# RazonIn4K/image-restoration-platform

Measured on AMD Instinct MI355X. Metric: restored images/sec @1024x1024 bs=8, higher is better.
Workload: dtype bf16; 1 GPU; 1024x1024 RGB u8, batch 8 per GPU: fused classifier scan + RestoreNet-v0 (43 convs, 779.9 GFLOP/image), seeded random-init weights; global_batch=8, parallelism=per-image data parallel x1, no collective, streams=1

## Files before the change

### image_restoration_platform_amd/csrc/conv_dnq.hip

```cpp
#include "conv_mfma.hpp"
#include "persist.hpp"

#include <type_traits>

namespace ire {

namespace {

typedef __bf16 bf16x8_t __attribute__((ext_vector_type(8)));
typedef __bf16 bf16x2_t __attribute__((ext_vector_type(2)));
typedef float f32x2_t __attribute__((ext_vector_type(2)));
typedef float f32x16_t __attribute__((ext_vector_type(16)));
typedef unsigned u32x4_t __attribute__((ext_vector_type(4)));

#ifndef DQ_ST
#define DQ_ST IRE_ST_LINE
#endif
#ifndef DQ_ABL
#define DQ_ABL 0
#endif

constexpr int DQ_THREADS = 512;
constexpr int DQ_TH = 16, DQ_TW = 32, DQ_IH = 17, DQ_IW = 33, DQ_NT = 128, DQ_NTL = 4;
constexpr int DQ_TILE_PIECES = 36;
// ... 42 lines not shown
}

template <int COUT>
__global__ __launch_bounds__(DQ_THREADS) void conv_dnq_kernel(ConvArgs a) {
    constexpr int NT = DQ_NT, NTL = DQ_NTL, C = COUT;
    __shared__ __attribute__((aligned(16))) unsigned char smem[DQ_LDS];
    const unsigned smem_lds = (unsigned)(size_t)(__attribute__((address_space(3))) unsigned char*)smem;
    const int tid = threadIdx.x;
    const int lane = tid & 63, wave = tid >> 6;
    const int r = lane & 31, h = lane >> 5;
    const int wv = __builtin_amdgcn_readfirstlane(wave);

    const int NKC = a.nkc;
    const int Cin = a.cin0;
    const int tiles_per_img = a.tiles_x * a.tiles_y;
    PersistCursor cursor(a.tiles_x, a.tiles_y, a.nimg, C / NT, 4 * NKC);
    const int n_items = cursor.my_items, S = cursor.S;
    if (S == 0) return;

    unsigned slotc[5];
#pragma unroll
    for (int d = 0; d < 5; ++d) {
        int l2 = lane;
        asm volatile("" : "+v"(l2));
        const int piece = d < 4 ? 4 * wv + d : 32 + (wv & 3);
        const int s = piece * 64 + l2, p = s >> 2, c8 = (s & 3) ^ ((p >> 2) & 3);
        const int py = p / DQ_IW, px = p - py * DQ_IW;
        slotc[d] = (unsigned)py | ((unsigned)px << 8) | ((unsigned)c8 << 16);
    }
    const char* const zeros = reinterpret_cast<const char*>(a.zeros);
    struct Plan { const void* src[10]; unsigned dst[10]; int n; };
// ... 256 lines not shown
```

### image_restoration_platform_amd/csrc/conv_down.hip

```cpp
#include "conv_mfma.hpp"
#include "persist.hpp"

namespace ire {

namespace {

typedef __bf16 bf16x8_t __attribute__((ext_vector_type(8)));
typedef __bf16 bf16x2_t __attribute__((ext_vector_type(2)));
typedef float f32x2_t __attribute__((ext_vector_type(2)));
typedef float f32x16_t __attribute__((ext_vector_type(16)));
typedef unsigned u32x4_t __attribute__((ext_vector_type(4)));

#ifndef DN_LD_NT
#define DN_LD_NT 0
#endif
constexpr int DN_THREADS = 512;
constexpr int DN_TH = 16, DN_TW = 32;
constexpr int DN_IH = DN_TH + 1, DN_IW = DN_TW + 1;
constexpr int DN_IN_CHUNKS = DN_IH * DN_IW * 4;
constexpr int DN_IN_ITERS = (DN_IN_CHUNKS + DN_THREADS - 1) / DN_THREADS;
constexpr int DN_IN_BYTES = DN_IN_ITERS * DN_THREADS * 16;
constexpr int DN_NT = 64, DN_NTL = 2;
constexpr int DN_W_BYTES_MAX = 4 * 4 * DN_NT * 16;
constexpr int DN_W_BASE = 2 * DN_IN_BYTES;
// ... 30 lines not shown
template <int N> __device__ __forceinline__ void dn_wait_vm(bool counted) {
    if (counted) asm volatile("s_waitcnt vmcnt(%0)" :: "n"(N) : "memory");
    else asm volatile("s_waitcnt vmcnt(0)" ::: "memory");
}

__global__ __launch_bounds__(DN_THREADS) void conv_down_kernel(ConvArgs a) {
    __shared__ __attribute__((aligned(16))) unsigned char smem[DN_LDS];
    const unsigned smem_lds = (unsigned)(size_t)(__attribute__((address_space(3))) unsigned char*)smem;
    const int tid = threadIdx.x;
    const int lane = tid & 63, wave = tid >> 6;
    const int r = lane & 31, h = lane >> 5;
    const int c8_fixed = tid & 3;

    const int tiles_per_img = a.tiles_x * a.tiles_y;
    const int nkc = a.nkc;
    PersistCursor cursor(a.tiles_x, a.tiles_y, a.nimg, a.nblocks, 4 * nkc);
    const int my_items = cursor.my_items;
    const int S = cursor.S;
    if (S == 0) return;
    using StageInfo = PersistStage;
    StageInfo sq0 = cursor.cur, sq1 = cursor.next(), sq2 = cursor.next();

    const int Cin = a.cin0;
    const int cin_shift = 31 - __builtin_clz(Cin);

    int a_off[2][4];
#pragma unroll
    for (int m = 0; m < 2; ++m)
#pragma unroll
        for (int o = 0; o < 4; ++o) {
            const int dy = (o >> 1) - 1, dx = (o & 1) - 1;
// ... 258 lines not shown
```

### image_restoration_platform_amd/csrc/conv_f8.hip

```cpp
#include "conv_mfma.hpp"
#include "persist.hpp"
#include "gn_fold.hpp"

namespace ire {

namespace {

typedef __bf16 bf16x2_t __attribute__((ext_vector_type(2)));
typedef float f32x2_t __attribute__((ext_vector_type(2)));
typedef float f32x16_t __attribute__((ext_vector_type(16)));
typedef unsigned u32x4_t __attribute__((ext_vector_type(4)));
typedef int i32x8_t __attribute__((ext_vector_type(8)));

constexpr float kF8ActScale = 16.0f;
constexpr int F8_THREADS = 512;
constexpr int F8_TH = 16, F8_TW = 32, F8_IH = 18, F8_IW = 34;
constexpr int F8_PX = F8_IH * F8_IW;
constexpr int F8_IN_CHUNKS = F8_PX * 4;
constexpr int F8_IN_ITERS = (F8_IN_CHUNKS + F8_THREADS - 1) / F8_THREADS;
constexpr int F8_PLANE = F8_PX * 16;
constexpr int F8_IN_BYTES = 2 * F8_PLANE + 64;
constexpr int F8_NT = 128, F8_NTL = 4;
constexpr int F8_W_BYTES = 9 * 2 * F8_NT * 16;
constexpr int F8_W_CHUNKS = F8_W_BYTES / 16;
// ... 35 lines not shown
}

struct F8Regs { uint4 v[F8_IN_ITERS]; unsigned ok; };

template <bool RESID>
__global__ __launch_bounds__(F8_THREADS) void conv_f8_kernel(ConvArgs a) {
    __shared__ __attribute__((aligned(16))) unsigned char smem[F8_LDS];
    const unsigned smem_lds = (unsigned)(size_t)(__attribute__((address_space(3))) unsigned char*)smem;
    const int tid = threadIdx.x;
    const int lane = tid & 63, wave = tid >> 6;
    const int r = lane & 31, h = lane >> 5;
    const int c8_fixed = tid & 3;

    const int tiles_per_img = a.tiles_x * a.tiles_y;
    const int nkc = a.nkc;
    PersistCursor cursor(a.tiles_x, a.tiles_y, a.nimg, a.nblocks, nkc);
    const int my_items = cursor.my_items;
    const int S = cursor.S;
    if (S == 0) return;
    if (a.gn_stats) gn_fold(a, smem, cursor.first_img, cursor.last_img);
    using StageInfo = PersistStage;
    StageInfo sq0 = cursor.cur, sq1 = cursor.next(), sq2 = cursor.next();

    const int Cin = a.cin0;
    const int cin_shift = 31 - __builtin_clz(Cin);

    int p_off[2][5], w_off[5];
#pragma unroll
    for (int i = 0; i < 5; ++i) {
        const int tap = min(2 * i + h, 8);
        const int ky = tap / 3, kx = tap - ky * 3;
// ... 291 lines not shown
```

### image_restoration_platform_amd/csrc/conv_mfma.hpp

```cpp
#pragma once
#include "common.hpp"
#include "conv_kind.hpp"

#ifndef IRE_ST_LINE
#define IRE_ST_LINE 16
#endif
#ifndef IRE_LD_ONCE
#define IRE_LD_ONCE 2
#endif
#ifndef IRE_LD_IN
#define IRE_LD_IN 0
#endif
#ifndef IRE_ST_PART
#define IRE_ST_PART 0
#endif

#include <cstdlib>

namespace ire {

inline int persistent_grid_cus() {
    static const int forced = [] { const char* v = std::getenv("IRE_GRID_CUS"); return v ? std::atoi(v) : 0; }();
    int dev = 0, cus = 256;
    (void)hipGetDevice(&dev);
// ... 25 lines not shown
    const unsigned char* u8_in;
    unsigned char* u8_out;
    float* stats;
    int Hin, Win, Hout, Wout, cout;
    int tiles_x, tiles_y, nimg, nblocks;
    int group_size;
    int prio_young;
    int in_rows;
    int in_row_off;
    int iy_lo, iy_span;
    int fp8;
    const float* oscale;
    int w4_nt;
    const void* zeros;
    unsigned long long* stamps;
};

void conv_launch(ConvKind kind, const ConvArgs& a, hipStream_t stream);

void conv_rb_launch(bool resid, bool fused_act, const ConvArgs& a, hipStream_t stream);
void conv_w4_launch(bool resid, const ConvArgs& a, hipStream_t stream);
void conv_f8_launch(bool resid, const ConvArgs& a, hipStream_t stream);
void conv_stem_launch(const ConvArgs& a, hipStream_t stream);
void conv_down_launch(const ConvArgs& a, hipStream_t stream);
void conv_head_launch(const ConvArgs& a, hipStream_t stream);
void conv_pc_launch(bool resid, bool head, const ConvArgs& a, hipStream_t stream);
void conv_pk_launch(bool resid, const ConvArgs& a, hipStream_t stream);
void conv_up_subpixel_launch(const ConvArgs& a, hipStream_t stream);
void conv_upq_launch(const ConvArgs& a, hipStream_t stream);
void conv_dnq_launch(const ConvArgs& a, hipStream_t stream);
// ... 4 lines not shown
```

### image_restoration_platform_amd/csrc/conv_pc.hip

```cpp
#include "conv_mfma.hpp"
#include "conv_plan.hpp"
#include "gn_fold.hpp"
#include "persist.hpp"

#include <type_traits>

namespace ire {

namespace {

typedef __bf16 bf16x8_t __attribute__((ext_vector_type(8)));
typedef __bf16 bf16x2_t __attribute__((ext_vector_type(2)));
typedef float f32x2_t __attribute__((ext_vector_type(2)));
typedef float f32x16_t __attribute__((ext_vector_type(16)));
typedef unsigned u32x4_t __attribute__((ext_vector_type(4)));

#ifndef C3_RES_PRE
#define C3_RES_PRE -1
#endif
#ifndef C3_SCALAR
#define C3_SCALAR 1
#endif
#ifndef C3_PRIO
#define C3_PRIO 1
// ... 89 lines not shown
        (void)k;
#endif
    };

    auto tl = [&](int slot) {
#ifdef IRE_W4_TL
        if (a.stamps && tid == 0) {
            a.stamps[(size_t)blockIdx.x * 32 + slot * 2] = __builtin_amdgcn_s_memrealtime();
            a.stamps[(size_t)blockIdx.x * 32 + slot * 2 + 1] = __builtin_amdgcn_s_memtime();
        }
#else
        (void)slot;
#endif
    };
    const int tiles_per_img = a.tiles_x * a.tiles_y;
    PersistCursor cursor(a.tiles_x, a.tiles_y, a.nimg, K::NBLK, NKC);
    const int n_items = cursor.my_items;
    if (n_items == 0) return;
    const int n_stages = n_items * NKC;
    tl(0);
    {
        const unsigned char* ws = reinterpret_cast<const unsigned char*>(a.w);
        const unsigned wl = (unsigned)(size_t)(__attribute__((address_space(3))) unsigned char*)smem + K::W_OFF;
        constexpr int PIECES = NKC * K::W_STAGE_CHUNKS / 64;
        static_assert((NKC * K::W_STAGE_CHUNKS) % 64 == 0, "whole wave-instructions");
        const int wv = __builtin_amdgcn_readfirstlane(wave);
        for (int p = wv; p < PIECES; p += THREADS / 64) c3_glds16(ws + ((size_t)p * 64 + lane) * 16, wl + p * 1024);
    }
    if (a.gn_stats) gn_fold(a, smem, cursor.first_img, cursor.last_img, 512, reinterpret_cast<float2*>(smem + K::COEF_OFF));
    tl(1);

// ... 606 lines not shown
```

### image_restoration_platform_amd/csrc/conv_pk.hip

```cpp
#include "conv_mfma.hpp"
#include "conv_plan.hpp"
#include "gn_fold.hpp"
#include "persist.hpp"

#include <type_traits>

namespace ire {

namespace {

typedef __bf16 bf16x8_t __attribute__((ext_vector_type(8)));
typedef __bf16 bf16x2_t __attribute__((ext_vector_type(2)));
typedef float f32x2_t __attribute__((ext_vector_type(2)));
typedef float f32x16_t __attribute__((ext_vector_type(16)));
typedef unsigned u32x4_t __attribute__((ext_vector_type(4)));

#ifndef PK_PRIO
#define PK_PRIO 1
#endif
#ifndef PK_DMA_SPLIT
#define PK_DMA_SPLIT 1
#endif
#ifndef PK_BDEPTH
#define PK_BDEPTH 2
// ... 73 lines not shown
    return x + y;
}
__device__ __forceinline__ void pk_barrier() { asm volatile("s_waitcnt lgkmcnt(0)\n\ts_barrier" ::: "memory"); }

template <int C, bool RESID>
__global__ __launch_bounds__(PK_THREADS) void conv_pk_kernel(ConvArgs a) {
    using K = PkCfg<C>;
    constexpr int NKC = C / 16, NBLK = C / PK_NT, NT = PK_NT, NTL = PK_NTL;
    __shared__ __attribute__((aligned(16))) unsigned char smem[K::LDS];
    const unsigned smem_lds = (unsigned)(size_t)(__attribute__((address_space(3))) unsigned char*)smem;
    const int tid = threadIdx.x;
    const int lane = tid & 63, wave = tid >> 6;
    const int r = lane & 31, h = lane >> 5;

    const int tiles_per_img = a.tiles_x * a.tiles_y;
    PersistCursor cursor(a.tiles_x, a.tiles_y, a.nimg, NBLK, NKC);
    const int n_items = cursor.my_items, S = cursor.S;
    if (S == 0) return;
    auto stamp = [&](int role, int stage, int k) {
#ifdef PK_TICKS
        if (a.stamps && lane == 0 && blockIdx.x < 8 && stage < 32) a.stamps[(((size_t)blockIdx.x * 2 + role) * 32 + stage) * 4 + k] = __builtin_amdgcn_s_memtime();
#else
        (void)role; (void)stage; (void)k;
#endif
    };
    auto tl = [&](int slot) {
#ifdef IRE_W4_TL
        if (a.stamps && tid == 0) {
            a.stamps[(size_t)blockIdx.x * 32 + slot * 2] = __builtin_amdgcn_s_memrealtime();
            a.stamps[(size_t)blockIdx.x * 32 + slot * 2 + 1] = __builtin_amdgcn_s_memtime();
        }
// ... 460 lines not shown
```

### image_restoration_platform_amd/csrc/conv_rb.hip

```cpp
#include "conv_mfma.hpp"
#include "persist.hpp"
#include "gn_fold.hpp"

#include <cstdlib>

namespace ire {

namespace {

typedef __bf16 bf16x8_t __attribute__((ext_vector_type(8)));
typedef __bf16 bf16x2_t __attribute__((ext_vector_type(2)));
typedef float f32x2_t __attribute__((ext_vector_type(2)));
typedef float f32x16_t __attribute__((ext_vector_type(16)));
typedef unsigned u32x4_t __attribute__((ext_vector_type(4)));

constexpr int RB_TH = kRbTileH, RB_TW = 32;
constexpr int RB_WAVES = RB_TH / 2;
constexpr int RB_THREADS = RB_WAVES * 64;
constexpr int RB_IH = RB_TH + 2, RB_IW = RB_TW + 2;
constexpr int RB_IN_CHUNKS = RB_IH * RB_IW * 4;
constexpr int RB_IN_ITERS = (RB_IN_CHUNKS + RB_THREADS - 1) / RB_THREADS;
constexpr int RB_IN_BYTES = RB_IN_ITERS * RB_THREADS * 16;
constexpr int RB_NSTEPS = 18;

// ... 70 lines not shown

    const unsigned smem_lds = (unsigned)(size_t)(__attribute__((address_space(3))) unsigned char*)smem;
    const int tid = threadIdx.x;
    const int lane = tid & 63, wave = tid >> 6;
    const int r = lane & 31, h = lane >> 5;
    const int c8_fixed = tid & 3;
    auto stamp = [&](int s, int k) {
        if constexpr (DBG & 16) {
            const unsigned long long t = __builtin_amdgcn_s_memtime();
            if (a.stamps && lane == 0 && (wave == 0 || wave == 4) && blockIdx.x < 8 && s < 64)
                a.stamps[(((size_t)blockIdx.x * 2 + (wave >> 2)) * 64 + s) * 10 + k] = t;
        }
    };

    const int tiles_per_img = a.tiles_x * a.tiles_y;
    PersistCursor cursor(a.tiles_x, a.tiles_y, a.nimg, a.nblocks, a.nkc);
    const int nkc = a.nkc;
    const int S = cursor.S;
    if (S == 0) return;
    if (a.gn_stats) gn_fold(a, smem, cursor.first_img, cursor.last_img);
    using StageInfo = PersistStage;
    StageInfo sq0 = cursor.cur, sq1 = cursor.next(), sq2 = cursor.next();

    const unsigned short* src = reinterpret_cast<const unsigned short*>(a.in0);
    const int Cin = a.cin0;

    int a_off[2][9];
#pragma unroll
    for (int m = 0; m < 2; ++m)
#pragma unroll
        for (int tap = 0; tap < 9; ++tap) {
// ... 482 lines not shown
```

### image_restoration_platform_amd/csrc/conv_stem.hip

```cpp
#include "conv_mfma.hpp"

#include <type_traits>

namespace ire {

namespace {

typedef __bf16 bf16x8_t __attribute__((ext_vector_type(8)));
typedef __bf16 bf16x2_t __attribute__((ext_vector_type(2)));
typedef float f32x2_t __attribute__((ext_vector_type(2)));
typedef float f32x16_t __attribute__((ext_vector_type(16)));
typedef unsigned u32x4_t __attribute__((ext_vector_type(4)));

constexpr int ST_THREADS = 512, ST_TH = 16, ST_TW = 32, ST_IH = ST_TH + 2, ST_IW = ST_TW + 2;
constexpr int ST_RB = ST_IW * 3;
constexpr int ST_PW = ST_IW + 2;
constexpr int ST_ROW = ST_PW * 4;
constexpr int ST_ITERS = (ST_IH * ST_RB + ST_THREADS - 1) / ST_THREADS;

__device__ __forceinline__ unsigned st_pack(float a, float b) {
    f32x2_t f = {a, b};
    return __builtin_bit_cast(unsigned, __builtin_convertvector(f, bf16x2_t));
}
template <int N> __device__ __forceinline__ float st_ror_add(float v) {
// ... 18 lines not shown
    f32x16_t bias_acc;
#pragma unroll
    for (int i = 0; i < 16; ++i) bias_acc[i] = a.bias[16 * (i >> 3) + 8 * h + (i & 7)];
    const int foff = (2 * wave * ST_PW + r + 2 * h) * 4;
    for (int i = tid; i < 2 * ST_IH * ST_ROW / 2; i += ST_THREADS) reinterpret_cast<unsigned*>(&tile[0][0])[i] = 0u;
    __syncthreads();
    int spy[ST_ITERS], sb[ST_ITERS], spx[ST_ITERS], srel[ST_ITERS];
#pragma unroll
    for (int it = 0; it < ST_ITERS; ++it) {
        const int i = tid + it * ST_THREADS;
        spy[it] = i / ST_RB; sb[it] = i - spy[it] * ST_RB;
        spx[it] = sb[it] / 3;
        srel[it] = (spy[it] * a.Win + spx[it]) * 3 + (sb[it] - spx[it] * 3);
    }

    const int tiles_per_img = a.tiles_x * a.tiles_y, total = tiles_per_img * a.nimg;
    const unsigned char* in = reinterpret_cast<const unsigned char*>(a.in0);
    const bf16x2_t ones = __builtin_bit_cast(bf16x2_t, 0x3f803f80u);
    unsigned pv[ST_ITERS];
    auto request = [&](int item) {
        const int img = item / tiles_per_img, t = item - img * tiles_per_img;
        const int ty = t / a.tiles_x, tx = t - ty * a.tiles_x;
        const int iy0 = ty * ST_TH - 1, ix0 = tx * ST_TW - 1;
        const long long base = (((long long)img * a.in_rows + iy0 + a.in_row_off) * a.Win + ix0) * 3;
#pragma unroll
        for (int it = 0; it < ST_ITERS; ++it) {
            const bool ok = spy[it] < ST_IH && (unsigned)(iy0 + spy[it] - a.iy_lo) < (unsigned)a.iy_span && (unsigned)(ix0 + spx[it]) < (unsigned)a.Win;
            const unsigned v = in[ok ? base + srel[it] : 0];
            pv[it] = ok ? v : 0u;
        }
    };
    int par = 0;
    if ((int)blockIdx.x < total) request(blockIdx.x);
    for (int item = blockIdx.x; item < total; item += gridDim.x) {
        const int img = item / tiles_per_img, t = item - img * tiles_per_img;
        const int ty = t / a.tiles_x, tx = t - ty * a.tiles_x;
        unsigned short* tl = tile[par];
#pragma unroll
        for (int it = 0; it < ST_ITERS; ++it)
            if (spy[it] < ST_IH) tl[spy[it] * ST_ROW + spx[it] * 4 + (sb[it] - spx[it] * 3)] = (unsigned short)(__builtin_bit_cast(unsigned, (float)pv[it]) >> 16);
        if (item + (int)gridDim.x < total) request(item + gridDim.x);
        __syncthreads();
        const int ox = tx * ST_TW + r;
        char* obase = reinterpret_cast<char*>(a.out) + (size_t)img * a.Hout * a.Wout * 64;
        float gs[2][2] = {{0.f, 0.f}, {0.f, 0.f}}, gq[2][2] = {{0.f, 0.f}, {0.f, 0.f}};
#pragma unroll
        for (int m = 0; m < 2; ++m) {
            u32x4_t f[3];
#pragma unroll
            for (int ky = 0; ky < 3; ++ky) {
                const uint2* fp = reinterpret_cast<const uint2*>(tl + foff + (m + ky) * ST_ROW);
                const uint2 lo = fp[0], hi = fp[1];
                f[ky] = u32x4_t{lo.x, lo.y, hi.x, hi.y};
            }
            f32x16_t c = __builtin_amdgcn_mfma_f32_32x32x16_bf16(w0, __builtin_bit_cast(bf16x8_t, f[0]), bias_acc, 0, 0, 0);
            c = __builtin_amdgcn_mfma_f32_32x32x16_bf16(w1, __builtin_bit_cast(bf16x8_t, f[1]), c, 0, 0, 0);
// ... 68 lines not shown
```

### image_restoration_platform_amd/csrc/conv_up.hip

```cpp
#include "conv_mfma.hpp"
#include "persist.hpp"

#include <type_traits>

namespace ire {

namespace {

typedef __bf16 bf16x8_t __attribute__((ext_vector_type(8)));
typedef __bf16 bf16x2_t __attribute__((ext_vector_type(2)));
typedef float f32x2_t __attribute__((ext_vector_type(2)));
typedef float f32x16_t __attribute__((ext_vector_type(16)));
typedef unsigned u32x4_t __attribute__((ext_vector_type(4)));

#ifndef IRE_UP_TEPI
#define IRE_UP_TEPI 1
#endif
#ifndef IRE_UP_ABL
#define IRE_UP_ABL 0
#endif
constexpr int UP_THREADS = 512;
constexpr int UP_TH = 16, UP_TW = 32;
constexpr int UP_IH = UP_TH + 2, UP_IW = UP_TW + 2;
constexpr int UP_IN_CHUNKS = UP_IH * UP_IW * 4;
// ... 35 lines not shown
    if constexpr (I < N) { f(std::integral_constant<int, I>{}); up_static_for<I + 1, N>(f); }
}

using UpItem = PersistItem;
struct UpRegs { uint4 v[UP_IN_ITERS]; };

template <int NKS>
__global__ __launch_bounds__(UP_THREADS) void conv_up_kernel(ConvArgs a) {
    __shared__ __attribute__((aligned(16))) unsigned char smem[UP_LDS];
    const unsigned smem_lds = (unsigned)(size_t)(__attribute__((address_space(3))) unsigned char*)smem;
    const int tid = threadIdx.x;
    const int lane = tid & 63, wave = tid >> 6;
    const int r = lane & 31, h = lane >> 5;
    const int c8_fixed = tid & 3;

    PersistCursor cursor(a.tiles_x, a.tiles_y, a.nimg, a.nblocks, a.nkc);
    const int my_items = cursor.my_items;
    const int nkc = a.nkc;
    const int S = cursor.S;
    if (S == 0) return;
    using StageInfo = PersistStage;
    StageInfo sq0 = cursor.cur, sq1 = cursor.next(), sq2 = cursor.next();

    const int Cin = a.cin0;
    const int cin_shift = 31 - __builtin_clz(Cin);

    int a_off[2][9];
#pragma unroll
    for (int m = 0; m < 2; ++m)
#pragma unroll
        for (int tap = 0; tap < 9; ++tap) {
// ... 466 lines not shown
```

### image_restoration_platform_amd/csrc/conv_upq.hip

```cpp
#include "conv_mfma.hpp"
#include "persist.hpp"

#include <type_traits>

namespace ire {

namespace {

typedef __bf16 bf16x8_t __attribute__((ext_vector_type(8)));
typedef __bf16 bf16x2_t __attribute__((ext_vector_type(2)));
typedef float f32x2_t __attribute__((ext_vector_type(2)));
typedef float f32x16_t __attribute__((ext_vector_type(16)));
typedef unsigned u32x4_t __attribute__((ext_vector_type(4)));

#ifndef UQ_ST
#define UQ_ST IRE_ST_LINE
#endif
#ifndef UQ_DMA_SPAN
#define UQ_DMA_SPAN 32
#endif
#ifndef UQ_ABL
#define UQ_ABL 0
#endif

// ... 35 lines not shown
}

__global__ __launch_bounds__(UQ_THREADS) void conv_upq_kernel(ConvArgs a) {
    constexpr int NT = UQ_NT, NTL = UQ_NTL, C = UQ_NT;
    __shared__ __attribute__((aligned(16))) unsigned char smem[UQ_LDS];
    const unsigned smem_lds = (unsigned)(size_t)(__attribute__((address_space(3))) unsigned char*)smem;
    const int tid = threadIdx.x;
    const int lane = tid & 63, wave = tid >> 6;
    const int r = lane & 31, h = lane >> 5;
    const int wv = __builtin_amdgcn_readfirstlane(wave);

    const int NKC = a.nkc;
    const int NST = NKC;
    const int Cin = a.cin0;
    const int tiles_per_img = a.tiles_x * a.tiles_y;
    PersistCursor cursor(a.tiles_x, a.tiles_y, a.nimg, 4, NST);
    const int n_items = cursor.my_items, S = cursor.S;
    if (S == 0) return;

    unsigned slotc[5];
#pragma unroll
    for (int d = 0; d < 5; ++d) {
        int l2 = lane;
        asm volatile("" : "+v"(l2));
        const int piece = d < 4 ? 4 * wv + d : 32 + (wv & 3);
        const int s = piece * 64 + l2, p = s >> 2, c8 = (s & 3) ^ ((p >> 2) & 3);
        const int py = p / UQ_IW, px = p - py * UQ_IW;
        slotc[d] = (unsigned)py | ((unsigned)px << 8) | ((unsigned)c8 << 16);
    }
    const char* const zeros = reinterpret_cast<const char*>(a.zeros);
    struct Plan { const void* src[10]; unsigned dst[10]; int n; };
// ... 276 lines not shown
```

### image_restoration_platform_amd/csrc/conv_w4.hip

```cpp
#include "conv_mfma.hpp"
#include "persist.hpp"
#include "gn_fold.hpp"

#include <cstdlib>
#include <type_traits>

#ifndef W4_TEPI
#define W4_TEPI 1
#endif

namespace ire {

namespace {

typedef __bf16 bf16x8_t __attribute__((ext_vector_type(8)));
typedef __bf16 bf16x2_t __attribute__((ext_vector_type(2)));
typedef float f32x2_t __attribute__((ext_vector_type(2)));
typedef float f32x16_t __attribute__((ext_vector_type(16)));

constexpr int W4_TH = 16, W4_TW = 32, W4_IH = 18, W4_IW = 34;
constexpr int W4_IN_CHUNKS = W4_IH * W4_IW * 2;
constexpr int W4_IN_BYTES = (W4_IN_CHUNKS + 8) * 16;
constexpr int W4_NSTEPS = 9;

// ... 59 lines not shown
__global__ __launch_bounds__(WAVES * 64) void conv_w4_kernel(ConvArgs a) {
    static_assert(!FP8 || (FUSED && WAVES == 8), "fp8 operands: fused-activation 8-wave form only");
    using C = W4Cfg<NT, WAVES, FP8>;
    constexpr int EB = C::EB;
    using Regs = W4Regs<C::IN_ITERS>;
    constexpr int NTL = C::NTL;
    __shared__ __attribute__((aligned(16))) unsigned char smem[C::LDS_BYTES];
    const unsigned smem_lds = (unsigned)(size_t)(__attribute__((address_space(3))) unsigned char*)smem;

    const int tid = threadIdx.x;
    const int lane = tid & 63, wave = tid >> 6;
    const int r = lane & 31, h = lane >> 5;
    const int c8_fixed = tid & 1;

    const int tiles_per_img = a.tiles_x * a.tiles_y;
    PersistCursor cursor(a.tiles_x, a.tiles_y, a.nimg, a.nblocks, a.nkc);
    const int my_items = cursor.my_items;
    const int nkc = a.nkc;
    const int S = cursor.S;
    if (S == 0) return;
#ifdef IRE_W4_TL
    if (a.stamps && tid == 0) { a.stamps[(size_t)blockIdx.x * 32] = __builtin_amdgcn_s_memrealtime(); a.stamps[(size_t)blockIdx.x * 32 + 1] = __builtin_amdgcn_s_memtime(); }
#endif
    using StageInfo = PersistStage;
    StageInfo sq0 = cursor.cur, sq1 = cursor.next(), sq2 = cursor.next();

    const int Cin = a.cin0;
    const int cin_shift = 31 - __builtin_clz(Cin);

    constexpr int PLANE = C::PLANE;
    const int a_base = h * PLANE + (wave * C::MT * W4_IW + r) * EB;
// ... 606 lines not shown
```

### image_restoration_platform_amd/csrc/engine.cpp

```cpp
#include "engine.hpp"
#include "encode.hpp"

#include <chrono>
#include <cmath>
#include <cstdlib>
#include <cstring>
#include <fstream>

#include "gn.hpp"
#include "strips.hpp"
#include "weight_pack.hpp"
#include "grey_tables.inc"

namespace ire {

namespace {

const int kWidths[4] = {32, 64, 128, 256};
const int kFilmOff[4] = {0, 64, 192, 448};
const int kFilmDim = 960;

inline double now_s() {
    return std::chrono::duration<double>(std::chrono::steady_clock::now().time_since_epoch()).count();
}
// ... 17 lines not shown
    hipDeviceProp_t prop;
    IRE_HIP(hipGetDeviceProperties(&prop, device_));
    if (std::strncmp(prop.gcnArchName, "gfx950", 6) != 0)
        fail(IRE_ERR_UNAVAILABLE, std::string("service unavailable: device is ") + prop.gcnArchName +
                                      ", this engine is built for gfx950 (MI355X) only");
    if (cfg.precision != IRE_PRECISION_BF16 && cfg.precision != IRE_PRECISION_FP8) fail(IRE_ERR_INVALID_INPUT, "invalid precision");
    precision_ = cfg.precision;
    max_batch_ = cfg.max_batch > 0 ? cfg.max_batch : 8;
    if (max_batch_ > 64) fail(IRE_ERR_INVALID_INPUT, "invalid max_batch (1..64)");
    num_lanes_ = cfg.num_streams > 0 ? cfg.num_streams : 1;
    if (num_lanes_ > 16) num_lanes_ = 16;
    if (cfg.flags & ~(uint32_t)IRE_FLAG_RESULT_PNG_BASE64) fail(IRE_ERR_INVALID_INPUT, "invalid ire_config.flags (unknown bits set)");
    flags_ = cfg.flags;
    sw_ = ConvSwitches::from_env();
    cus_ = persistent_grid_cus();
    if (const char* v = std::getenv("IRE_RB_STAMPS")) {
        stamps_cout_ = std::atoi(v);
        stamps_resid_ = std::strchr(v, 'r') != nullptr;
    }
    if (const char* v = std::getenv("IRE_W4_TL")) stamps_tl_ = v;

    IRE_HIP(hipStreamCreateWithFlags(&main_stream_, hipStreamNonBlocking));
    for (auto& ev : ev_) IRE_HIP(hipEventCreate(&ev));
    IRE_HIP(hipEventCreateWithFlags(&fork_ev_, hipEventDisableTiming));
    IRE_HIP(hipEventCreateWithFlags(&busy_ev_, hipEventDisableTiming));
    lanes_.resize(num_lanes_);
    for (auto& L : lanes_) {
        IRE_HIP(hipStreamCreateWithFlags(&L.stream, hipStreamNonBlocking));
        IRE_HIP(hipEventCreateWithFlags(&L.done, hipEventDisableTiming));
    }
// ... 538 lines not shown
    a.cin0 = d.cin0; a.cin1 = p.cin1; a.kc_split = d.kc_split; a.nkc = p.nkc; a.nblocks = p.nblocks; a.w4_nt = p.w4_nt; a.fp8 = p.fp8;
    const unsigned short* const slabs[] = {nullptr, cw.d_w, cw.d_wp, cw.d_w4, cw.d_w4h, cw.d_wstem, cw.d_wd, cw.d_wu, cw.d_wuf, cw.d_wdq, cw.d_wuq, cw.d_wsq,
                                           cw.d_wsk, reinterpret_cast<const unsigned short*>(cw.d_w8x), reinterpret_cast<const unsigned short*>(cw.d_w8)};
    const float* const biases[] = {cw.d_bias, cw.d_bias_uf, cw.d_bias8};
    a.w = slabs[p.w]; a.w1 = slabs[p.w1]; a.bias = biases[p.bias];
    if (p.fp8) a.oscale = cw.d_oscale;
    if (p.zeros) a.zeros = d_zero_;
    a.ab = op.use_ab ? R.ab : nullptr; a.resid = out_ptr(op.resid); a.out = out_ptr(op.out);
    a.u8_in = d.kind == CONV_HEAD ? g.img_in + (size_t)g.halo * g.w * 3 : nullptr;
    a.u8_out = d.kind == CONV_HEAD ? g.img_out : nullptr;
    a.Hin = g.h >> op.lin; a.Win = g.w >> op.lin; a.Hout = Hout; a.Wout = Wout;
    a.in_rows = p.in_rows; a.in_row_off = p.in_row_off; a.iy_lo = p.iy_lo; a.iy_span = p.iy_span;
    a.cout = p.cout; a.group_size = p.group_size; a.tiles_x = p.tiles_x; a.tiles_y = p.tiles_y; a.nimg = g.nimg;
    if (op.stats_out) a.stats = (R.stats_alt ? R.stats_alt : R.stats) + p.stats_offset();
    a.prio_young = sw_.prio_young;
    const bool rb = d.kind == CONV_RB1 || d.kind == CONV_RB2;
    if (stamps_dev_ && rb && d.cout == stamps_cout_ && (d.kind == CONV_RB2) == stamps_resid_ && (!stamps_taken_ || !stamps_tl_.empty() || std::getenv("IRE_STAMPS_RAW"))) {
        a.stamps = stamps_dev_;
        stamps_taken_ = true;
    }
    if (R.gn_pending) {
        if (p.folds_gn) {
            const GNW& gn = *R.gn_pending;
            a.gn_stats = R.gn_stats; a.gn_parts = R.gn_parts; a.gn_hw = (g.H >> gn.level) * (g.w >> gn.level);
            a.gn_gamma = gn.d_gamma; a.gn_beta = gn.d_beta; a.gn_film = R.film; a.gn_film_stride = kFilmDim; a.gn_film_off = kFilmOff[gn.level];
            a.ab_w = R.ab;
            R.gn_pending = nullptr;
        } else flush_gn(R, g);
    }
    prof_begin(p.fam, R.stream, p.flops, p.bytes);
// ... 36 lines not shown

void Engine::exec_op(Run& R, const Op& op, const Geo& g) {
    switch (op.kind) {
        case Op::GN: {
            R.gn_pending = op.gn; R.gn_stats = R.stats; R.gn_parts = R.stat_parts;
            if (!sw_.gn_fold || g.halo) flush_gn(R, g);
            break;
        }
        case Op::CONV: exec_conv(R, op, g); break;
    }
}

void Engine::run_network(Lane& L, int nimg, int h, int w, const uint8_t* d_in, uint8_t* d_out, const float* d_film) {
    Run R;
    R.stream = L.stream; R.stats = L.stats; R.stats_alt = L.stats2; R.ab = L.ab; R.film = d_film;
    const Geo g = geo_of_lane(L, nimg, h, w, d_in, d_out);
    prof_chain_ = false;
    prof_chainable_ = capture_ == false;
    prof_skip_ = prof_on_ == 2 && prof_every_ > 1 && (prof_pass_ % prof_every_) != 0;
    ++prof_pass_;
    for (const Op& op : program_) exec_op(R, op, g);
    prof_chainable_ = false;
    prof_chain_ = false;
    prof_skip_ = false;
}

void Engine::classify_device(const uint8_t* d_rgb, int n, int h, int w, const uint8_t* d_is_jpeg, double* d_scores,
                             int32_t* d_label, hipStream_t stream) {
    check_shape(n, h, w, false);
    if (!d_rgb) fail(IRE_ERR_INVALID_INPUT, "invalid input: null image pointer");
// ... 214 lines not shown
```

### image_restoration_platform_amd/csrc/engine.hpp

```cpp
#pragma once
#include <deque>
#include <map>
#include <mutex>
#include <string>
#include <vector>

#include "classifier.hpp"
#include "common.hpp"
#include "conv_mfma.hpp"
#include "conv_plan.hpp"

namespace ire {

struct PackedConv;
struct ConvW {
    ConvDesc desc;
    unsigned short* d_w = nullptr;
    unsigned short* d_wp = nullptr;
    unsigned short* d_w4 = nullptr;
    unsigned short* d_w4h = nullptr;
    unsigned short* d_wstem = nullptr;
    unsigned short* d_wd = nullptr;
    unsigned short* d_wu = nullptr;
    unsigned short* d_wuf = nullptr;
// ... 49 lines not shown
    bool use_ab = false;
    bool halo_out = false;
    bool stats_out = false;
    std::string name;
};
struct Run {
    hipStream_t stream = nullptr;
    float* stats = nullptr;
    float2* ab = nullptr;
    const float* film = nullptr;
    int stat_parts = 0;
    float* stats_alt = nullptr;
    const GNW* gn_pending = nullptr;
    const float* gn_stats = nullptr;
    int gn_parts = 0;
};
struct Geo {
    int nimg = 1, h = 0, w = 0;
    int halo = 0;
    bool has_up = false, has_down = false;
    int y0 = 0, H = 0;
    unsigned short* buf[4][6] = {};
    const uint8_t* img_in = nullptr;
    uint8_t* img_out = nullptr;
};

struct ProfRec {
    int fam;
    bool own_e0 = true;
    hipEvent_t e0, e1;
// ... 93 lines not shown
    void prof_tag(const char* key, const char* kernel, int level, int cin, int cout, double flops_exec);
    void prof_end(hipStream_t s);
    void capture(const char* name, const unsigned short* d, size_t count, hipStream_t s);
    void capture_f32(const char* name, const float* d, size_t count, hipStream_t s);
    template <class T> T* upload(const std::vector<T>& v);
    ConvW upload_conv(const PackedConv& p);
    void* dalloc(size_t bytes);

    int device_ = 0;
    int max_batch_ = 8;
    int num_lanes_ = 1;
    uint32_t flags_ = 0;
    int precision_ = IRE_PRECISION_BF16;
    ConvSwitches sw_;
    int cus_ = 256;
    std::mutex mu_;
    hipStream_t main_stream_ = nullptr;
    hipEvent_t ev_[4] = {};
    hipEvent_t fork_ev_ = nullptr;
    hipEvent_t busy_ev_ = nullptr;
    bool busy_recorded_ = false;
    int64_t batches_run_ = 0, images_restored_ = 0;
    int last_batch_ = 0;
    std::deque<std::pair<double, int>> recent_;
    double t0_ = 0.0;

    ClassifierTables tables_{};
    std::vector<void*> table_allocs_;

    size_t io_cap_imgs_ = 0, io_cap_px_ = 0;
// ... 64 lines not shown
```

### image_restoration_platform_amd/csrc/persist.hpp

```cpp
#pragma once

namespace ire {

struct PersistItem { int img, ty, tx, nb, tile; };
struct PersistStage { PersistItem it; int kc; };

struct PersistCursor {
    int S;
    int my_items;
    int nkc, nblocks, tiles_x, tiles_y;
    int d_img, d_ty, d_tx, d_nb;
    int s;
    PersistStage cur;
    int first_img, last_img;

    __device__ __forceinline__ PersistCursor(int tiles_x_, int tiles_y_, int nimg, int nblocks_, int nkc_) {
        tiles_x = tiles_x_; tiles_y = tiles_y_; nblocks = nblocks_; nkc = nkc_;
        const int tiles_per_img = tiles_x * tiles_y;
        const int items = tiles_per_img * nimg * nblocks;
        const int G = gridDim.x;
        const int X = G < 8 ? G : 8;
        const int xcd = blockIdx.x % X, jx = blockIdx.x / X;
        const int nwx = (G - xcd + X - 1) / X;
        const int lo = (int)((long long)items * xcd / X), hi = (int)((long long)items * (xcd + 1) / X);
        my_items = (lo + jx < hi) ? (hi - lo - jx + nwx - 1) / nwx : 0;
        S = my_items * nkc;
        auto split = [&](int L, int& img, int& ty, int& tx, int& nb) {
            nb = L % nblocks;
            const int t = L / nblocks;
            img = t / tiles_per_img;
            const int tile = t - img * tiles_per_img;
            ty = tile / tiles_x;
            tx = tile - ty * tiles_x;
        };
        split(nwx, d_img, d_ty, d_tx, d_nb);
        split(lo + jx, cur.it.img, cur.it.ty, cur.it.tx, cur.it.nb);
        cur.it.tile = cur.it.ty * tiles_x + cur.it.tx;
        cur.kc = 0;
        s = 0;
        first_img = cur.it.img;
        last_img = my_items > 0 ? (lo + jx + (my_items - 1) * nwx) / nblocks / tiles_per_img : first_img;
    }
    __device__ __forceinline__ PersistStage next() {
        if (s + 1 < S) {
            ++s;
            if (++cur.kc == nkc) {
                cur.kc = 0;
                PersistItem& it = cur.it;
                it.nb += d_nb;
                int c = 0;
                if (it.nb >= nblocks) { it.nb -= nblocks; c = 1; }
                it.tx += d_tx + c; c = 0;
                if (it.tx >= tiles_x) { it.tx -= tiles_x; c = 1; }
                it.ty += d_ty + c; c = 0;
                if (it.ty >= tiles_y) { it.ty -= tiles_y; c = 1; }
                it.img += d_img + c;
                it.tile = it.ty * tiles_x + it.tx;
            }
// ... 7 lines not shown
```

Baseline: 1110 images/sec.

## Alternate persistent tile walk direction between consecutive convs for cache reuse

Adds a reverse-walk mode to the persistent work cursor and alternates forward and reverse traversal between successive conv launches (a snake order), enabled by default via IRE_SNAKE. The idea is that the tiles a block finishes with in one layer are still resident in L2/MALL when the next layer starts on the same region, cutting DRAM traffic for activations. The stem kernel is moved onto the shared cursor so it can take part. The reverse-stride arithmetic with carries is intricate, so any error would skip or duplicate tiles.

```diff
diff --git a/image_restoration_platform_amd/csrc/conv_dnq.hip b/image_restoration_platform_amd/csrc/conv_dnq.hip
--- a/image_restoration_platform_amd/csrc/conv_dnq.hip
+++ b/image_restoration_platform_amd/csrc/conv_dnq.hip
@@ -80,7 +80,7 @@
     const int NKC = a.nkc;
     const int Cin = a.cin0;
     const int tiles_per_img = a.tiles_x * a.tiles_y;
-    PersistCursor cursor(a.tiles_x, a.tiles_y, a.nimg, C / NT, 4 * NKC);
+    PersistCursor cursor(a.tiles_x, a.tiles_y, a.nimg, C / NT, 4 * NKC, (int)gridDim.x, (int)blockIdx.x, a.walk_rev != 0);
     const int n_items = cursor.my_items, S = cursor.S;
     if (S == 0) return;
 
diff --git a/image_restoration_platform_amd/csrc/conv_down.hip b/image_restoration_platform_amd/csrc/conv_down.hip
--- a/image_restoration_platform_amd/csrc/conv_down.hip
+++ b/image_restoration_platform_amd/csrc/conv_down.hip
@@ -68,7 +68,7 @@
 
     const int tiles_per_img = a.tiles_x * a.tiles_y;
     const int nkc = a.nkc;
-    PersistCursor cursor(a.tiles_x, a.tiles_y, a.nimg, a.nblocks, 4 * nkc);
+    PersistCursor cursor(a.tiles_x, a.tiles_y, a.nimg, a.nblocks, 4 * nkc, (int)gridDim.x, (int)blockIdx.x, a.walk_rev != 0);
     const int my_items = cursor.my_items;
     const int S = cursor.S;
     if (S == 0) return;
diff --git a/image_restoration_platform_amd/csrc/conv_f8.hip b/image_restoration_platform_amd/csrc/conv_f8.hip
--- a/image_restoration_platform_amd/csrc/conv_f8.hip
+++ b/image_restoration_platform_amd/csrc/conv_f8.hip
@@ -73,7 +73,7 @@
 
     const int tiles_per_img = a.tiles_x * a.tiles_y;
     const int nkc = a.nkc;
-    PersistCursor cursor(a.tiles_x, a.tiles_y, a.nimg, a.nblocks, nkc);
+    PersistCursor cursor(a.tiles_x, a.tiles_y, a.nimg, a.nblocks, nkc, (int)gridDim.x, (int)blockIdx.x, a.walk_rev != 0);
     const int my_items = cursor.my_items;
     const int S = cursor.S;
     if (S == 0) return;
diff --git a/image_restoration_platform_amd/csrc/conv_mfma.hpp b/image_restoration_platform_amd/csrc/conv_mfma.hpp
--- a/image_restoration_platform_amd/csrc/conv_mfma.hpp
+++ b/image_restoration_platform_amd/csrc/conv_mfma.hpp
@@ -63,6 +63,7 @@
     int w4_nt;
     const void* zeros;
     unsigned long long* stamps;
+    int walk_rev;
 };
 
 void conv_launch(ConvKind kind, const ConvArgs& a, hipStream_t stream);
diff --git a/image_restoration_platform_amd/csrc/conv_pc.hip b/image_restoration_platform_amd/csrc/conv_pc.hip
--- a/image_restoration_platform_amd/csrc/conv_pc.hip
+++ b/image_restoration_platform_amd/csrc/conv_pc.hip
@@ -127,7 +127,7 @@
 #endif
     };
     const int tiles_per_img = a.tiles_x * a.tiles_y;
-    PersistCursor cursor(a.tiles_x, a.tiles_y, a.nimg, K::NBLK, NKC);
+    PersistCursor cursor(a.tiles_x, a.tiles_y, a.nimg, K::NBLK, NKC, (int)gridDim.x, (int)blockIdx.x, a.walk_rev != 0);
     const int n_items = cursor.my_items;
     if (n_items == 0) return;
     const int n_stages = n_items * NKC;
diff --git a/image_restoration_platform_amd/csrc/conv_pk.hip b/image_restoration_platform_amd/csrc/conv_pk.hip
--- a/image_restoration_platform_amd/csrc/conv_pk.hip
+++ b/image_restoration_platform_amd/csrc/conv_pk.hip
@@ -111,7 +111,7 @@
     const int r = lane & 31, h = lane >> 5;
 
     const int tiles_per_img = a.tiles_x * a.tiles_y;
-    PersistCursor cursor(a.tiles_x, a.tiles_y, a.nimg, NBLK, NKC);
+    PersistCursor cursor(a.tiles_x, a.tiles_y, a.nimg, NBLK, NKC, (int)gridDim.x, (int)blockIdx.x, a.walk_rev != 0);
     const int n_items = cursor.my_items, S = cursor.S;
     if (S == 0) return;
     auto stamp = [&](int role, int stage, int k) {
diff --git a/image_restoration_platform_amd/csrc/conv_rb.hip b/image_restoration_platform_amd/csrc/conv_rb.hip
--- a/image_restoration_platform_amd/csrc/conv_rb.hip
+++ b/image_restoration_platform_amd/csrc/conv_rb.hip
@@ -108,7 +108,7 @@
     };
 
     const int tiles_per_img = a.tiles_x * a.tiles_y;
-    PersistCursor cursor(a.tiles_x, a.tiles_y, a.nimg, a.nblocks, a.nkc);
+    PersistCursor cursor(a.tiles_x, a.tiles_y, a.nimg, a.nblocks, a.nkc, (int)gridDim.x, (int)blockIdx.x, a.walk_rev != 0);
     const int nkc = a.nkc;
     const int S = cursor.S;
     if (S == 0) return;
diff --git a/image_restoration_platform_amd/csrc/conv_stem.hip b/image_restoration_platform_amd/csrc/conv_stem.hip
--- a/image_restoration_platform_amd/csrc/conv_stem.hip
+++ b/image_restoration_platform_amd/csrc/conv_stem.hip
@@ -1,4 +1,5 @@
 #include "conv_mfma.hpp"
+#include "persist.hpp"
 
 #include <type_traits>
 
@@ -56,15 +57,13 @@
         srel[it] = (spy[it] * a.Win + spx[it]) * 3 + (sb[it] - spx[it] * 3);
     }
 
-    const int tiles_per_img = a.tiles_x * a.tiles_y, total = tiles_per_img * a.nimg;
+    const int tiles_per_img = a.tiles_x * a.tiles_y;
     const unsigned char* in = reinterpret_cast<const unsigned char*>(a.in0);
     const bf16x2_t ones = __builtin_bit_cast(bf16x2_t, 0x3f803f80u);
     unsigned pv[ST_ITERS];
-    auto request = [&](int item) {
-        const int img = item / tiles_per_img, t = item - img * tiles_per_img;
-        const int ty = t / a.tiles_x, tx = t - ty * a.tiles_x;
-        const int iy0 = ty * ST_TH - 1, ix0 = tx * ST_TW - 1;
-        const long long base = (((long long)img * a.in_rows + iy0 + a.in_row_off) * a.Win + ix0) * 3;
+    auto request = [&](const PersistItem& ri) {
+        const int iy0 = ri.ty * ST_TH - 1, ix0 = ri.tx * ST_TW - 1;
+        const long long base = (((long long)ri.img * a.in_rows + iy0 + a.in_row_off) * a.Win + ix0) * 3;
 #pragma unroll
         for (int it = 0; it < ST_ITERS; ++it) {
             const bool ok = spy[it] < ST_IH && (unsigned)(iy0 + spy[it] - a.iy_lo) < (unsigned)a.iy_span && (unsigned)(ix0 + spx[it]) < (unsigned)a.Win;
@@ -73,15 +72,17 @@
         }
     };
     int par = 0;
-    if ((int)blockIdx.x < total) request(blockIdx.x);
-    for (int item = blockIdx.x; item < total; item += gridDim.x) {
-        const int img = item / tiles_per_img, t = item - img * tiles_per_img;
-        const int ty = t / a.tiles_x, tx = t - ty * a.tiles_x;
+    PersistCursor cursor(a.tiles_x, a.tiles_y, a.nimg, 1, 1, (int)gridDim.x, (int)blockIdx.x, a.walk_rev != 0);
+    const int n_items = cursor.my_items;
+    PersistItem nx = cursor.cur.it;
+    if (n_items > 0) request(nx);
+    for (int k = 0; k < n_items; ++k) {
+        const int img = nx.img, t = nx.tile, ty = nx.ty, tx = nx.tx;
         unsigned short* tl = tile[par];
 #pragma unroll
         for (int it = 0; it < ST_ITERS; ++it)
             if (spy[it] < ST_IH) tl[spy[it] * ST_ROW + spx[it] * 4 + (sb[it] - spx[it] * 3)] = (unsigned short)(__builtin_bit_cast(unsigned, (float)pv[it]) >> 16);
-        if (item + (int)gridDim.x < total) request(item + gridDim.x);
+        if (k + 1 < n_items) { nx = cursor.next().it; request(nx); }
         __syncthreads();
         const int ox = tx * ST_TW + r;
         char* obase = reinterpret_cast<char*>(a.out) + (size_t)img * a.Hout * a.Wout * 64;
diff --git a/image_restoration_platform_amd/csrc/conv_up.hip b/image_restoration_platform_amd/csrc/conv_up.hip
--- a/image_restoration_platform_amd/csrc/conv_up.hip
+++ b/image_restoration_platform_amd/csrc/conv_up.hip
@@ -73,7 +73,7 @@
     const int r = lane & 31, h = lane >> 5;
     const int c8_fixed = tid & 3;
 
-    PersistCursor cursor(a.tiles_x, a.tiles_y, a.nimg, a.nblocks, a.nkc);
+    PersistCursor cursor(a.tiles_x, a.tiles_y, a.nimg, a.nblocks, a.nkc, (int)gridDim.x, (int)blockIdx.x, a.walk_rev != 0);
     const int my_items = cursor.my_items;
     const int nkc = a.nkc;
     const int S = cursor.S;
diff --git a/image_restoration_platform_amd/csrc/conv_upq.hip b/image_restoration_platform_amd/csrc/conv_upq.hip
--- a/image_restoration_platform_amd/csrc/conv_upq.hip
+++ b/image_restoration_platform_amd/csrc/conv_upq.hip
@@ -73,7 +73,7 @@
     const int NST = NKC;
     const int Cin = a.cin0;
     const int tiles_per_img = a.tiles_x * a.tiles_y;
-    PersistCursor cursor(a.tiles_x, a.tiles_y, a.nimg, 4, NST);
+    PersistCursor cursor(a.tiles_x, a.tiles_y, a.nimg, 4, NST, (int)gridDim.x, (int)blockIdx.x, a.walk_rev != 0);
     const int n_items = cursor.my_items, S = cursor.S;
     if (S == 0) return;
 
diff --git a/image_restoration_platform_amd/csrc/conv_w4.hip b/image_restoration_platform_amd/csrc/conv_w4.hip
--- a/image_restoration_platform_amd/csrc/conv_w4.hip
+++ b/image_restoration_platform_amd/csrc/conv_w4.hip
@@ -97,7 +97,7 @@
     const int c8_fixed = tid & 1;
 
     const int tiles_per_img = a.tiles_x * a.tiles_y;
-    PersistCursor cursor(a.tiles_x, a.tiles_y, a.nimg, a.nblocks, a.nkc);
+    PersistCursor cursor(a.tiles_x, a.tiles_y, a.nimg, a.nblocks, a.nkc, (int)gridDim.x, (int)blockIdx.x, a.walk_rev != 0);
     const int my_items = cursor.my_items;
     const int nkc = a.nkc;
     const int S = cursor.S;
diff --git a/image_restoration_platform_amd/csrc/engine.cpp b/image_restoration_platform_amd/csrc/engine.cpp
--- a/image_restoration_platform_amd/csrc/engine.cpp
+++ b/image_restoration_platform_amd/csrc/engine.cpp
@@ -55,6 +55,7 @@
     flags_ = cfg.flags;
     sw_ = ConvSwitches::from_env();
     cus_ = persistent_grid_cus();
+    if (const char* v = std::getenv("IRE_SNAKE")) snake_ = std::atoi(v) != 0;
     if (const char* v = std::getenv("IRE_RB_STAMPS")) {
         stamps_cout_ = std::atoi(v);
         stamps_resid_ = std::strchr(v, 'r') != nullptr;
@@ -623,6 +624,8 @@
     a.cout = p.cout; a.group_size = p.group_size; a.tiles_x = p.tiles_x; a.tiles_y = p.tiles_y; a.nimg = g.nimg;
     if (op.stats_out) a.stats = (R.stats_alt ? R.stats_alt : R.stats) + p.stats_offset();
     a.prio_young = sw_.prio_young;
+    a.walk_rev = R.snake && R.next_rev && p.kernel != K_V1;
+    R.next_rev = !a.walk_rev;
     const bool rb = d.kind == CONV_RB1 || d.kind == CONV_RB2;
     if (stamps_dev_ && rb && d.cout == stamps_cout_ && (d.kind == CONV_RB2) == stamps_resid_ && (!stamps_taken_ || !stamps_tl_.empty() || std::getenv("IRE_STAMPS_RAW"))) {
         a.stamps = stamps_dev_;
@@ -689,6 +692,7 @@
 void Engine::run_network(Lane& L, int nimg, int h, int w, const uint8_t* d_in, uint8_t* d_out, const float* d_film) {
     Run R;
     R.stream = L.stream; R.stats = L.stats; R.stats_alt = L.stats2; R.ab = L.ab; R.film = d_film;
+    R.snake = snake_;
     const Geo g = geo_of_lane(L, nimg, h, w, d_in, d_out);
     prof_chain_ = false;
     prof_chainable_ = capture_ == false;
diff --git a/image_restoration_platform_amd/csrc/engine.hpp b/image_restoration_platform_amd/csrc/engine.hpp
--- a/image_restoration_platform_amd/csrc/engine.hpp
+++ b/image_restoration_platform_amd/csrc/engine.hpp
@@ -87,6 +87,8 @@
     const GNW* gn_pending = nullptr;
     const float* gn_stats = nullptr;
     int gn_parts = 0;
+    bool snake = false;
+    bool next_rev = false;
 };
 struct Geo {
     int nimg = 1, h = 0, w = 0;
@@ -210,6 +212,7 @@
     int precision_ = IRE_PRECISION_BF16;
     ConvSwitches sw_;
     int cus_ = 256;
+    bool snake_ = true;
     std::mutex mu_;
     hipStream_t main_stream_ = nullptr;
     hipEvent_t ev_[4] = {};
diff --git a/image_restoration_platform_amd/csrc/persist.hpp b/image_restoration_platform_amd/csrc/persist.hpp
--- a/image_restoration_platform_amd/csrc/persist.hpp
+++ b/image_restoration_platform_amd/csrc/persist.hpp
@@ -1,4 +1,10 @@
 #pragma once
+
+#if defined(__HIPCC__) || defined(__CUDACC__)
+#define IRE_HD __host__ __device__ __forceinline__
+#else
+#define IRE_HD inline
+#endif
 
 namespace ire {
 
@@ -14,13 +20,12 @@
     PersistStage cur;
     int first_img, last_img;
 
-    __device__ __forceinline__ PersistCursor(int tiles_x_, int tiles_y_, int nimg, int nblocks_, int nkc_) {
+    IRE_HD PersistCursor(int tiles_x_, int tiles_y_, int nimg, int nblocks_, int nkc_, int G, int block, bool reverse) {
         tiles_x = tiles_x_; tiles_y = tiles_y_; nblocks = nblocks_; nkc = nkc_;
         const int tiles_per_img = tiles_x * tiles_y;
         const int items = tiles_per_img * nimg * nblocks;
-        const int G = gridDim.x;
         const int X = G < 8 ? G : 8;
-        const int xcd = blockIdx.x % X, jx = blockIdx.x / X;
+        const int xcd = block % X, jx = block / X;
         const int nwx = (G - xcd + X - 1) / X;
         const int lo = (int)((long long)items * xcd / X), hi = (int)((long long)items * (xcd + 1) / X);
         my_items = (lo + jx < hi) ? (hi - lo - jx + nwx - 1) / nwx : 0;
@@ -34,14 +39,21 @@
             tx = tile - ty * tiles_x;
         };
         split(nwx, d_img, d_ty, d_tx, d_nb);
-        split(lo + jx, cur.it.img, cur.it.ty, cur.it.tx, cur.it.nb);
+        const int L_lo = lo + jx, span = my_items > 0 ? (my_items - 1) * nwx : 0;
+        split(reverse ? L_lo + span : L_lo, cur.it.img, cur.it.ty, cur.it.tx, cur.it.nb);
         cur.it.tile = cur.it.ty * tiles_x + cur.it.tx;
         cur.kc = 0;
         s = 0;
-        first_img = cur.it.img;
-        last_img = my_items > 0 ? (lo + jx + (my_items - 1) * nwx) / nblocks / tiles_per_img : first_img;
+        const int t_tx = d_tx + (d_nb ? 1 : 0), t_ty = d_ty + (t_tx ? 1 : 0);
+        d_img = reverse ? -d_img - (t_ty ? 1 : 0) : d_img;
+        d_ty = reverse && t_ty ? tiles_y - t_ty : reverse ? 0 : d_ty;
+        d_tx = reverse && t_tx ? tiles_x - t_tx : reverse ? 0 : d_tx;
+        d_nb = reverse && d_nb ? nblocks - d_nb : d_nb;
+        const int other_img = (reverse ? L_lo : L_lo + span) / nblocks / tiles_per_img;
+        first_img = reverse ? other_img : cur.it.img;
+        last_img = reverse ? cur.it.img : other_img;
     }
-    __device__ __forceinline__ PersistStage next() {
+    IRE_HD PersistStage next() {
         if (s + 1 < S) {
             ++s;
             if (++cur.kc == nkc) {
```

Measured after the change: 1131 images/sec, median of 6. +1.8%, better.
